# AkshayJha22/Cross-Sectional-Momentum-Strategy-Replication-Backtesting-Framework

Hardware: AMD Instinct MI355X
Metric: asset-periods backtested/sec (1/2/4/8 GPU) + % HBM peak BW; decile match % (higher is better)
Workload: dtype f64

## Files before the change

cross-sectional-momentum-strategy-replication-backtesting-framework_amd/csrc/scan.h:

```cpp
#pragma once
#include "csm_common.h"

struct ScanLane {
  double pff;
  double psff;
  int head;
  int prev;
};

__device__ __forceinline__ void scan_init(ScanLane& s, double* ring, int RS, int W,
                                          const double* __restrict__ carry, int64_t N,
                                          int64_t a, bool live) {
  if (live && carry) {
    for (int k = 0; k < W; ++k) ring[k * RS] = carry[(int64_t)k * N + a];
    s.pff = carry[(int64_t)W * N + a];
    s.psff = carry[(int64_t)(W + 1) * N + a];
  } else {
    for (int k = 0; k < W; ++k) ring[k * RS] = qnan();
    s.pff = qnan();
    s.psff = qnan();
  }
  s.head = 0;
  s.prev = -1;
}

__device__ __forceinline__ double ffill(double x, double last) { return isnan_d(x) ? last : x; }

__device__ __forceinline__ double price_step(double x, double& pff) {
  const double nx = ffill(x, pff);
  const double ret = nx / pff - 1.0;
  pff = nx;
  return ret;
}

__device__ __forceinline__ void lds_push(double* ring, int RS, int W, int& head, double fct) {
  ring[head * RS] = fct;
  head = (head + 1 == W) ? 0 : head + 1;
}

template <int JC = 0>
__device__ __forceinline__ double lds_prod(const double* ring, int RS, int W, int J, int idx) {
  double acc = ring[idx * RS];
  if constexpr (JC > 0) {
    double f[JC];
#pragma unroll
    for (int k = 1; k < JC; ++k) {
      idx = (idx + 1 == W) ? 0 : idx + 1;
      f[k] = ring[idx * RS];
    }
#pragma unroll
    for (int k = 1; k < JC; ++k) acc = acc * f[k];
  } else {
    for (int k = 1; k < J; ++k) {
      idx = (idx + 1 == W) ? 0 : idx + 1;
      acc = acc * ring[idx * RS];
    }
  }
  return acc;
}

template <int RW>
__device__ __forceinline__ void reg_push(double (&f)[RW], double fct, bool on = true) {
#pragma unroll
  for (int k = 0; k + 1 < RW; ++k) f[k] = on ? f[k + 1] : f[k];
  f[RW - 1] = on ? fct : f[RW - 1];
}

template <int RW>
__device__ __forceinline__ double reg_prod(const double (&f)[RW], int J) {
  double acc = f[0];
#pragma unroll
  for (int k = 1; k < RW; ++k)
    if (k < J) acc = acc * f[k];
  return acc;
}

template <int RW, bool FIX>
__device__ __forceinline__ double mj_window(const double (&f)[RW], int q, int lo, int hi) {
  if constexpr (FIX) {
    constexpr int Jq[4] = {3, 6, 9, 12};
    double acc = 0.0;
#pragma unroll
    for (int qq = 0; qq < 4; ++qq) {
      if (qq != q) continue;
      const int l = RW - Jq[qq] - 1;
      double a = f[l];
#pragma unroll
      for (int k = l + 1; k < RW - 1; ++k) a = a * f[k];
      acc = a;
    }
    return acc;
  }
  double acc = 1.0;
#pragma unroll
  for (int k = 0; k < RW; ++k) acc = (k >= lo && k < hi) ? acc * f[k] : acc;
  return acc;
}

__device__ __forceinline__ double subset_ret(double ps_new, double psff) {
  return ps_new / psff - 1.0;
}

template <class Settle>
__device__ __forceinline__ bool rank_step(double x, double mom, int m, double& psff, int& prev,
                                          Settle settle) {
  const bool ranked = !isnan_d(mom);
  const double ps_new = ffill(x, psff);
  if (prev >= 0) settle(prev, subset_ret(ps_new, psff));
  if (ranked) {
    psff = ps_new;
    prev = m;
    return false;
  }
  prev = -1;
  return true;
}

__device__ __forceinline__ double pending_finish(double x, double psff) {
  return is_absent(x) ? qnan() : subset_ret(ffill(x, psff), psff);
}

__device__ __forceinline__ void scan_finish(ScanLane& s, double* ring, int RS, int W, int64_t N,
                                            int64_t a, double* __restrict__ NR,
                                            const double* __restrict__ next_pm,
                                            double* __restrict__ carry_out) {
  if (s.prev >= 0)
    NR[(int64_t)s.prev * N + a] = next_pm ? pending_finish(next_pm[a], s.psff) : qnan();
  if (carry_out) {
    int idx = s.head;
    for (int k = 0; k < W; ++k) {
      carry_out[(int64_t)k * N + a] = ring[idx * RS];
      idx = (idx + 1 == W) ? 0 : idx + 1;
    }
    carry_out[(int64_t)W * N + a] = s.pff;
    carry_out[(int64_t)(W + 1) * N + a] = s.psff;
  }
}

template <int JC = 0>
__device__ __forceinline__ double lds_push_mom(ScanLane& s, double* ring, int RS, int W, int J,
                                               double fct) {
  lds_push(ring, RS, W, s.head, fct);
  return lds_prod<JC>(ring, RS, W, J, s.head) - 1.0;
}

template <class Ring>
__device__ __forceinline__ double scan_step_on(ScanLane& s, double x, int m, int64_t N, int64_t a,
                                               double* __restrict__ R, double* __restrict__ M,
                                               double* __restrict__ NR, Ring push_prod) {
  const double NaN = qnan();
  const int64_t o = (int64_t)m * N + a;
  if (is_absent(x)) {
    if (R) R[o] = NaN;
    M[o] = NaN;
    NR[o] = NaN;
    return NaN;
  }
  const double ret = price_step(x, s.pff);
  const double mom = push_prod(1.0 + ret);
  if (rank_step(x, mom, m, s.psff, s.prev,
                [&](int row, double nr) { NR[(int64_t)row * N + a] = nr; }))
    NR[o] = NaN;
  if (R) R[o] = ret;
  M[o] = mom;
  return mom;
}

__device__ __forceinline__ void store_pair(double* p, double v0, double v1) {
  *reinterpret_cast<double2*>(p) = make_double2(v0, v1);
}

__device__ __forceinline__ void store_next_ret_pair(double* __restrict__ NR, int64_t N,
                                                    int64_t a0, int64_t o, const int (&wp)[2],
                                                    const double (&vp)[2], const bool (&wc)[2]) {
  const double NaN = qnan();
  if (wp[0] >= 0 && wp[0] == wp[1]) {
    store_pair(NR + (int64_t)wp[0] * N + a0, vp[0], vp[1]);
  } else {
    if (wp[0] >= 0) NR[(int64_t)wp[0] * N + a0] = vp[0];
    if (wp[1] >= 0) NR[(int64_t)wp[1] * N + a0 + 1] = vp[1];
  }
  if (wc[0] && wc[1]) {
    store_pair(NR + o, NaN, NaN);
  } else {
    if (wc[0]) NR[o] = NaN;
    if (wc[1]) NR[o + 1] = NaN;
  }
}

__device__ __forceinline__ void chunk_range(int T_m, int G, int g, int& m0, int& m1) {
  const int base = T_m / G, rem = T_m % G;
  m0 = g * base + (g < rem ? g : rem);
  m1 = m0 + base + (g < rem ? 1 : 0);
}

template <int JC = 0>
__device__ __forceinline__ double scan_step(ScanLane& s, double x, int m, double* ring, int RS,
                                            int W, int J, int64_t N, int64_t a,
                                            double* __restrict__ R, double* __restrict__ M,
                                            double* __restrict__ NR) {
  return scan_step_on(s, x, m, N, a, R, M, NR,
                      [&](double fct) { return lds_push_mom<JC>(s, ring, RS, W, J, fct); });
}

template <int JC = 0>
__device__ __forceinline__ void scan_step_pair(ScanLane (&s)[2], const double (&x)[2], int m,
                                               double* ring0, int RS, int W, int J, int64_t N,
                                               int64_t a0, double* __restrict__ R,
                                               double* __restrict__ M, double* __restrict__ NR,
                                               double (&mom)[2]) {
  const double NaN = qnan();
  double ret[2];
  int wp[2];
  double vp[2];
  bool wc[2];
#pragma unroll
  for (int c = 0; c < 2; ++c) {
    wp[c] = -1;
    vp[c] = NaN;
    if (is_absent(x[c])) {
      ret[c] = NaN; mom[c] = NaN; wc[c] = true;
      continue;
    }
    ret[c] = price_step(x[c], s[c].pff);
    mom[c] = lds_push_mom<JC>(s[c], ring0 + c, RS, W, J, 1.0 + ret[c]);
    const bool ranked = !isnan_d(mom[c]);
    const double ps_new = ffill(x[c], s[c].psff);
    if (s[c].prev >= 0) { wp[c] = s[c].prev; vp[c] = subset_ret(ps_new, s[c].psff); }
    if (ranked) {
      s[c].psff = ps_new;
      s[c].prev = m;
      wc[c] = false;
    } else {
      s[c].prev = -1;
      wc[c] = true;
    }
  }
  const int64_t o = (int64_t)m * N + a0;
  if (R) store_pair(R + o, ret[0], ret[1]);
  store_pair(M + o, mom[0], mom[1]);
  store_next_ret_pair(NR, N, a0, o, wp, vp, wc);
}

__device__ __forceinline__ void scan_shadow(ScanLane& s, double x, int m, double* ring, int RS,
                                            int W, int J) {
  if (is_absent(x)) return;
  const double ret = price_step(x, s.pff);
  const double mom = lds_push_mom(s, ring, RS, W, J, 1.0 + ret);
  rank_step(x, mom, m, s.psff, s.prev, [](int, double) {});
}

template <int VEC> struct RowT;
template <> struct RowT<1> { typedef double T; };
template <> struct RowT<2> { typedef double2 T; };
__device__ __forceinline__ double comp(double v, int) { return v; }
__device__ __forceinline__ double comp(double2 v, int k) { return k == 0 ? v.x : v.y; }

template <int WR, int JC = 0>
__device__ __forceinline__ double scan_step_reg(ScanLane& s, double x, int m, double (&fr)[WR],
                                                int J, int64_t N, int64_t a,
                                                double* __restrict__ R, double* __restrict__ M,
                                                double* __restrict__ NR) {
  return scan_step_on(s, x, m, N, a, R, M, NR, [&](double fct) {
    reg_push(fr, fct);
    return reg_prod(fr, JC > 0 ? JC : J) - 1.0;
  });
}
```

cross-sectional-momentum-strategy-replication-backtesting-framework_amd/csrc/signal.hip:

```cpp
#include "csm_common.h"
#include "scan.h"
#include "shard.h"


#define PROBE_M 8
#define PROBE_DEN 8
__device__ __forceinline__ bool tail_probe(const double* __restrict__ P,
                                           const int64_t* __restrict__ month_start, int T_m,
                                           int64_t N, int64_t T_d) {
  static_assert(PROBE_M == 8, "the month spacing is a shift");
  const int lane = threadIdx.x & 63;
  const int64_t cs = N / 128;
  double x[PROBE_M][2];
  bool in[PROBE_M];
#pragma unroll
  for (int i = 0; i < PROBE_M; ++i) {
    const int m = (int)(((int64_t)(2 * i + 1) * T_m) >> 4);
    const int64_t d0 = month_start[m] < 0 ? 0 : month_start[m];
    const int64_t d1 = month_start[m + 1] < T_d ? month_start[m + 1] : T_d;
    in[i] = d1 > d0;
#pragma unroll
    for (int j = 0; j < 2; ++j)
      x[i][j] = in[i] ? P[(d1 - 1) * N + (2 * lane + j) * cs] : 0.0;
  }
  int gaps = 0, tot = 0;
#pragma unroll
  for (int i = 0; i < PROBE_M; ++i)
#pragma unroll
    for (int j = 0; j < 2; ++j) {
      gaps += __popcll(__ballot(in[i] && !(x[i][j] == x[i][j])));
      tot += in[i] ? 64 : 0;
    }
  return gaps * PROBE_DEN <= tot;
}

struct HaloArgs {
  int H, F, before, after;
  uint8_t* flags;
};
#define HALO_BATCH 8
template <int MAXD, int VEC, int NBUF, int BW, bool SH, bool BL, int JC = 0, bool HALO = false>
__global__ __launch_bounds__(64 * BW) void k_signal(
    const double* __restrict__ P, const int64_t* __restrict__ month_start, int T_m, int64_t N,
    int J, int skip, double* __restrict__ PMo, double* __restrict__ R, double* __restrict__ M,
    double* __restrict__ NR, const double* __restrict__ carry, const double* __restrict__ next_pm,
    double* __restrict__ carry_out, int64_t T_d, uint16_t* __restrict__ IDS, HaloArgs ha,
    int probe) {
  static_assert(!HALO || (SH && VEC == 2), "the halo prologue: shard passes, paired lanes");
  if (probe && tail_probe(P, month_start, T_m, N, T_d)) return;
  typedef typename RowT<VEC>::T VT;
  extern __shared__ __attribute__((aligned(16))) double ring_lds[];
  const int W = J + skip;
  const int tid = threadIdx.x;
  const int64_t a0 = ((int64_t)blockIdx.x * 64 * BW + tid) * VEC;
  const bool live = a0 < N;
  const int RS = 64 * VEC * BW;
  ScanLane sl[VEC];
  int* shc = reinterpret_cast<int*>(ring_lds + W * RS);
#pragma unroll
  for (int k = 0; k < VEC; ++k) {
    scan_init(sl[k], ring_lds + VEC * tid + k, RS, W, HALO ? nullptr : carry, N, a0 + k, live);
    if (SH) {
      shc[VEC * tid + k] = 0;
      shc[RS + VEC * tid + k] = -1;
      shc[2 * RS + VEC * tid + k] = -1;
    }
  }
  double npmh[VEC];
  if constexpr (HALO) {
    constexpr int HU = HALO_BATCH;
    const int64_t* ms = month_start;
    const int H = ha.H, F = ha.F, HF = H + F;
    const int64_t as = live ? a0 : 0;
    const int lane = tid & 63, wv = tid >> 6;
    const int64_t aw = a0 - 2 * lane;
    double* hpw = ring_lds + (size_t)W * RS + (size_t)(3 * RS) / 2;
    uint16_t* wl = reinterpret_cast<uint16_t*>(hpw + HU * RS) + wv * (HU * 128);
    int nh[VEC], fv[VEC], lv[VEC];
#pragma unroll
    for (int c = 0; c < VEC; ++c) { nh[c] = 0; fv[c] = -1; lv[c] = -1; npmh[c] = absent_val(); }
    for (int j0 = 0; j0 < HF; j0 += HU) {
      double2 xl[HU];
#pragma unroll
      for (int u = 0; u < HU; ++u) {
        const int j = j0 + u;
        const int m = j < H ? j : j + T_m;
        xl[u] = make_double2(absent_val(), absent_val());
        if (j < HF) {
          const int64_t d0 = ms[m], d1 = ms[m + 1];
          if (d1 > d0) xl[u] = *reinterpret_cast<const double2*>(P + (d1 - 1) * N + as);
        }
      }
      int nit = 0;
#pragma unroll
      for (int u = 0; u < HU; ++u) {
        *reinterpret_cast<double2*>(hpw + u * RS + 2 * tid) = xl[u];
#pragma unroll
        for (int c = 0; c < VEC; ++c) {
          const double x = comp(xl[u], c);
          const bool need = live && j0 + u < HF && !(x == x);
          const uint64_t mk = __ballot(need);
          if (need) wl[nit + lane_prefix(mk)] = (uint16_t)(u * 128 + 2 * lane + c);
          nit += __popcll(mk);
        }
      }
      __builtin_amdgcn_wave_barrier();
      for (int it0 = 0; it0 < nit; it0 += 128) {
        int item[2], u[2];
        int64_t d0[2], d1[2];
        double xs[2][HALO_WALK];
#pragma unroll
        for (int h = 0; h < 2; ++h) {
          const int it = it0 + 64 * h + lane;
          item[h] = it < nit ? (int)wl[it] : -1;
          u[h] = item[h] >> 7;
          const int j = j0 + (item[h] < 0 ? 0 : u[h]);
          const int m = j < H ? j : j + T_m;
          d0[h] = ms[m];
          d1[h] = ms[m + 1];
          const int64_t a = aw + (item[h] & 127);
#pragma unroll
          for (int k = 0; k < HALO_WALK; ++k) {
            const int64_t d = d1[h] - 2 - k;
            xs[h][k] = (item[h] >= 0 && d >= d0[h]) ? P[d * N + a] : absent_val();
          }
        }
#pragma unroll
        for (int h = 0; h < 2; ++h) {
          if (item[h] < 0) continue;
          const int64_t a = aw + (item[h] & 127);
          const double xlast = hpw[u[h] * RS + 128 * wv + (item[h] & 127)];
          bool p = !is_absent(xlast), got = false;
          double x = 0.0;
#pragma unroll
          for (int k = 0; k < HALO_WALK; ++k) {
            if (!got && xs[h][k] == xs[h][k]) { x = xs[h][k]; got = true; }
            p |= !is_absent(xs[h][k]);
          }
          if (!got && d1[h] - 1 - HALO_WALK > d0[h]) {
            const double y = halo_month_price(P, d0[h], d1[h] - 1 - HALO_WALK, N, a);
            if (y == y) { x = y; got = true; }
            p |= !is_absent(y);
          }
          hpw[u[h] * RS + 128 * wv + (item[h] & 127)] = got ? x : (p ? qnan() : absent_val());
        }
      }
      __syncthreads();
#pragma unroll
      for (int u = 0; u < HU; ++u) {
        const int j = j0 + u;
        if (j >= HF) break;
#pragma unroll
        for (int c = 0; c < VEC; ++c) {
          const double x = hpw[u * RS + 2 * tid + c];
          if (j < H) {
            if (live && !is_absent(x)) {
              if (!isnan_d(x)) { if (fv[c] < 0) fv[c] = nh[c]; lv[c] = nh[c]; }
              ++nh[c];
              scan_shadow(sl[c], x, j, ring_lds + VEC * tid + c, RS, W, J);
            }
          } else if (is_absent(npmh[c])) {
            npmh[c] = x;
          }
        }
      }
      __syncthreads();
    }
#pragma unroll
    for (int c = 0; c < VEC; ++c) {
      sl[c].prev = -1;
      uint8_t fl = 0;
      if (ha.before && !(fv[c] >= 0 && lv[c] - fv[c] >= W)) fl |= 1;
      if (ha.after && is_absent(npmh[c])) fl |= 2;
      if (live && ha.flags) ha.flags[a0 + c] = fl;
    }
    month_start += H;
  }
  const double* base = P + (live ? a0 : 0);
  const int64_t rstride = N;
  static_assert(!BL || VEC == 2, "buffer loads: paired lanes");
  const int voff = (int)((live ? a0 : 0) * 8);
  auto load_month = [&](VT (&buf)[MAXD], int mm) {
    mm = mm < T_m ? mm : T_m - 1;
    const int64_t f0 = month_start[mm], nn = month_start[mm + 1] - f0;
    if constexpr (BL) {
      typedef unsigned int u32x4 __attribute__((ext_vector_type(4)));
      const __amdgpu_buffer_rsrc_t rs = __builtin_amdgcn_make_buffer_rsrc(
          (void*)(P + f0 * N), (short)0, (int)(nn * N * 8), 0x00020000);
#pragma unroll
      for (int k = 0; k < MAXD; ++k) {
        const u32x4 w = __builtin_amdgcn_raw_buffer_load_b128(rs, voff + k * (int)(N * 8), 0, 0);
        buf[k] = *reinterpret_cast<const VT*>(&w);
      }
    } else {
      const int64_t pad = nn > 0 ? nn - 1 : (f0 > 0 ? -1 : 0);
#pragma unroll
      for (int k = 0; k < MAXD; ++k)
        buf[k] = *reinterpret_cast<const VT*>(base + (f0 + (k < nn ? k : pad)) * rstride);
    }
  };
  auto process = [&](const VT (&X)[MAXD], int m) {
    double pm[VEC];
    const int nnm = (int)(month_start[m + 1] - month_start[m]);
#pragma unroll
    for (int c = 0; c < VEC; ++c) {
      double last = 0.0;
      bool p = false, v = false;
#pragma unroll
      for (int k = 0; k < MAXD; ++k) {
        const double x = comp(X[k], c);
        const bool in = BL ? k < nnm : nnm > 0;
        const bool ok = in && x == x;
        p |= in && !is_absent(x);
        v |= ok;
        last = ok ? x : last;
      }
      pm[c] = p ? (v ? last : qnan()) : absent_val();
      if (SH && p) {
        int* q = shc + VEC * tid + c;
        q[0] += 1;
        if (q[RS] < 0) q[RS] = m;
        q[2 * RS] = m;
      }
    }
    if (live) {
      if (PMo && (!SH || shard_pm_kept(m, T_m, W))) {
        if (VEC == 2) *reinterpret_cast<double2*>(PMo + (int64_t)m * N + a0) = make_double2(pm[0], pm[VEC - 1]);
        else PMo[(int64_t)m * N + a0] = pm[0];
      }
      double mom[VEC];
      if constexpr (VEC == 2) {
        scan_step_pair<JC>(reinterpret_cast<ScanLane (&)[2]>(sl), reinterpret_cast<const double (&)[2]>(pm),
                       m, ring_lds + VEC * tid, RS, W, J, N, a0, R, M, NR,
                       reinterpret_cast<double (&)[2]>(mom));
      } else {
#pragma unroll
        for (int c = 0; c < VEC; ++c)
          mom[c] = scan_step(sl[c], pm[c], m, ring_lds + VEC * tid + c, RS, W, J, N, a0 + c, R, M, NR);
      }
      if (IDS) {
        if (VEC == 2)
          *reinterpret_cast<uint32_t*>(IDS + (int64_t)m * N + a0) =
              csm_fid(mom[0]) | (csm_fid(mom[VEC - 1]) << 16);
        else
          IDS[(int64_t)m * N + a0] = (uint16_t)csm_fid(mom[0]);
      }
    }
  };
  static_assert(NBUF == 2 || NBUF == 4, "two or four month buffers");
  VT A[MAXD], B[MAXD];
  if (NBUF == 2) {
    load_month(A, 0);
    for (int m = 0; m < T_m; m += 2) {
      load_month(B, m + 1);
      process(A, m);
      load_month(A, m + 2);
      if (m + 1 < T_m) process(B, m + 1);
    }
  } else {
    VT C[MAXD], D[MAXD];
    load_month(A, 0);
    load_month(B, 1);
    load_month(C, 2);
    for (int m = 0; m < T_m; m += 4) {
      load_month(D, m + 3);
      process(A, m);
      load_month(A, m + 4);
      if (m + 1 < T_m) process(B, m + 1);
      load_month(B, m + 5);
      if (m + 2 < T_m) process(C, m + 2);
      load_month(C, m + 6);
      if (m + 3 < T_m) process(D, m + 3);
    }
  }
  if (live) {
#pragma unroll
    for (int k = 0; k < VEC; ++k) {
      if constexpr (HALO) {
        if (sl[k].prev >= 0)
          NR[(int64_t)sl[k].prev * N + a0 + k] = pending_finish(npmh[k], sl[k].psff);
      } else {
        scan_finish(sl[k], ring_lds + VEC * tid + k, RS, W, N, a0 + k, NR, next_pm,
                    SH ? nullptr : carry_out);
      }
      if (SH) {
        const int* q = shc + VEC * tid + k;
        carry_out[a0 + k] = (double)q[0];
        carry_out[N + a0 + k] = (double)sl[k].prev;
        carry_out[2 * N + a0 + k] = sl[k].psff;
        carry_out[3 * N + a0 + k] = (double)q[RS];
        carry_out[4 * N + a0 + k] = (double)q[2 * RS];
      }
    }
  }
}

#define TAIL_U 8
#define TAIL_BACK 3

template <int MAXD, int BW, int JC>
__global__ __launch_bounds__(64 * BW) void k_signal_tail(
    const double* __restrict__ P, const int64_t* __restrict__ month_start, int T_m, int64_t N,
    int J, int skip, double* __restrict__ PMo, double* __restrict__ R, double* __restrict__ M,
    double* __restrict__ NR, const double* __restrict__ carry, const double* __restrict__ next_pm,
    double* __restrict__ carry_out, int64_t T_d, uint16_t* __restrict__ IDS,
    int probe) {
  if (probe && !tail_probe(P, month_start, T_m, N, T_d)) return;
  extern __shared__ __attribute__((aligned(16))) double ring_lds[];
  constexpr int U = TAIL_U, RS = 64 * BW, WA = 64;
  const int W = J + skip;
  const int tid = threadIdx.x, lane = tid & 63, wv = tid >> 6;
  const int64_t a0 = (int64_t)blockIdx.x * RS + tid;
  const bool live = a0 < N;
  const int64_t as = live ? a0 : 0;
  const int64_t aw = a0 - lane;
  const int64_t* ms = month_start;
  double* hp = ring_lds + (size_t)W * RS;
  double* hpw = hp + WA * wv;
  uint16_t* wl = reinterpret_cast<uint16_t*>(hp + U * RS) + wv * (2 * U * WA);
  uint16_t* wl2 = wl + U * WA;
  ScanLane sl;
  scan_init(sl, ring_lds + tid, RS, W, carry, N, a0, live);
  if (aw >= N) return;

  auto month_rows = [&](int m, int64_t& d0, int64_t& d1) {
    d0 = ms[m];
    d1 = ms[m + 1];
    d0 = d0 < 0 ? 0 : d0;
    d1 = d1 < T_d ? d1 : T_d;
  };
  auto load_last = [&](double (&xl)[U], int m0) {
#pragma unroll
    for (int u = 0; u < U; ++u) {
      xl[u] = absent_val();
      if (m0 + u < T_m) {
        int64_t d0, d1;
        month_rows(m0 + u, d0, d1);
        if (d1 > d0) xl[u] = P[(d1 - 1) * N + as];
      }
    }
  };
  auto fold = [&](double y, double& x, bool& got, bool& p) {
    if (!got && y == y) { x = y; got = true; }
    p |= !is_absent(y);
  };
  constexpr int K = MAXD - 1;
  struct Walk {
    int item, u, col;
    int64_t d0, d1;
    bool act;
  };
  auto issue = [&](auto& xs, Walk& w, const uint16_t* list, int it, int n, int m0) {
    constexpr int KK = sizeof(xs) / sizeof(double);
    w.act = it < n;
    w.item = w.act ? (int)list[it] : 0;
    w.u = w.item / WA;
    w.col = w.item % WA;
    month_rows(m0 + w.u, w.d0, w.d1);
    const int64_t a = aw + w.col;
#pragma unroll
    for (int k = 0; k < KK; ++k) {
      const int64_t d = w.d1 - 2 - k;
      xs[k] = (w.act && d >= w.d0) ? P[d * N + a] : absent_val();
    }
  };
  auto finish_back = [&](const double (&xs)[TAIL_BACK], const Walk& w, int& nb) {
    bool p = true, got = false;
    double x = 0.0;
#pragma unroll
    for (int k = 0; k < TAIL_BACK; ++k) fold(xs[k], x, got, p);
    const bool more = w.act && !got && w.d1 - 2 - TAIL_BACK >= w.d0;
    if (w.act && !more) hpw[w.u * RS + w.col] = got ? x : qnan();
    const uint64_t mk = __ballot(more);
    if (more) wl2[nb + lane_prefix(mk)] = (uint16_t)w.item;
    nb += __popcll(mk);
  };
  auto finish_month = [&](const double (&xs)[K], const Walk& w) {
    bool p = !is_absent(hpw[w.u * RS + w.col]), got = false;
    double x = 0.0;
#pragma unroll
    for (int k = 0; k < K; ++k) fold(xs[k], x, got, p);
    if (w.act) hpw[w.u * RS + w.col] = got ? x : (p ? qnan() : absent_val());
  };
  auto walk_months = [&](int i0, int n, int m0) {
    double XS[K], XT[K];
    Walk wb, wc;
    const bool two = i0 + 64 < n;
    issue(XS, wb, wl2, i0 + lane, n, m0);
    if (two) issue(XT, wc, wl2, i0 + 64 + lane, n, m0);
    finish_month(XS, wb);
    if (two) finish_month(XT, wc);
  };

  double xa[U], xb[U];
  load_last(xa, 0);
  for (int m0 = 0; m0 < T_m; m0 += U) {
    load_last(xb, m0 + U);
    int na = 0, nb = 0;
#pragma unroll
    for (int u = 0; u < U; ++u) {
      hp[u * RS + tid] = xa[u];
      bool in = false;
      if (m0 + u < T_m) {
        int64_t d0, d1;
        month_rows(m0 + u, d0, d1);
        in = d1 > d0;
      }
      const double x = xa[u];
      const bool need = live && in && !(x == x);
      const bool nb_ = need && is_absent(x), na_ = need && !nb_;
      const uint64_t mka = __ballot(na_), mkb = __ballot(nb_);
      const int item = u * WA + lane;
      if (na_) wl[na + lane_prefix(mka)] = (uint16_t)item;
      if (nb_) wl2[nb + lane_prefix(mkb)] = (uint16_t)item;
      na += __popcll(mka);
      nb += __popcll(mkb);
    }
    __builtin_amdgcn_wave_barrier();
    if (na + nb > 0) {
      double xs[TAIL_BACK];
      Walk wa;
      int db = nb < 128 ? nb : 128;
      issue(xs, wa, wl, lane, na, m0);
      walk_months(0, db, m0);
      finish_back(xs, wa, nb);
      for (int it0 = 64; it0 < na; it0 += 64) {
        issue(xs, wa, wl, it0 + lane, na, m0);
        finish_back(xs, wa, nb);
      }
      __builtin_amdgcn_wave_barrier();
      for (; db < nb; db += 128) walk_months(db, nb, m0);
    }
    __builtin_amdgcn_wave_barrier();
#pragma unroll 1
    for (int u = 0; u < U; ++u) {
      const int m = m0 + u;
      if (m >= T_m) break;
      if (!live) continue;
      const double pm = hp[u * RS + tid];
      if (PMo) PMo[(int64_t)m * N + a0] = pm;
      const double mom = scan_step<JC>(sl, pm, m, ring_lds + tid, RS, W, J, N, a0, R, M, NR);
      if (IDS) IDS[(int64_t)m * N + a0] = (uint16_t)csm_fid(mom);
    }
    __builtin_amdgcn_wave_barrier();
#pragma unroll
    for (int u = 0; u < U; ++u) xa[u] = xb[u];
  }
  if (live) scan_finish(sl, ring_lds + tid, RS, W, N, a0, NR, next_pm, carry_out);
}

static int g_tune_signal_vec = 2;
static int g_tune_signal_bwf = 0;
static int g_tune_signal_tail = 2;
static int g_tune_signal_j12 = 1;
#define SIGNAL_BWF_MIN_N (180 * 512)
static const TuneKnob g_knobs[] = {
    {"signal_vec", &g_tune_signal_vec, [](int v) { return v == 1 || v == 2; }},
    {"signal_bwf", &g_tune_signal_bwf, [](int v) { return v == 0 || v == 1 || v == 4; }},
    {"signal_j12", &g_tune_signal_j12, [](int v) { return v == 0 || v == 1; }},
    {"signal_tail", &g_tune_signal_tail, [](int v) { return v >= 0 && v <= 2; }},
};
int csm_tune_signal(const char* key, int value) { return tune_set(g_knobs, key, value); }

int signal_launch(csm_ctx* ctx, const char* who, const double* P, int64_t T_d, int64_t N,
                  const int64_t* month_start, int32_t T_m, int32_t max_month_days, int32_t J,
                  int32_t skip, double* PM, double* R, double* M, double* NR, const double* carry,
                  const double* next_pm, double* carry_out, bool sh, uint16_t* ids,
                  const HaloArgs* halo) {
  int r = prep(ctx);
  if (r) return r;
  if (sh && (!PM || !carry_out || T_m < 1))
    return set_err(ctx, CSM_E_INVAL, "%s: a shard pass needs PM and state, and at least one month",
                   who);
  if (!P || !month_start || !M || !NR || N <= 0 || T_d < 0 || T_m < 0 || J < 1 || skip < 0 ||
      J + skip > 256 || max_month_days < 1)
    return set_err(ctx, CSM_E_INVAL, "%s: bad arguments (N=%lld T_m=%d J=%d skip=%d)", who,
                   (long long)N, T_m, J, skip);
  if (max_month_days > 32)
    return set_err(ctx, CSM_E_INVAL, "%s: months longer than 32 days are not supported "
                   "(use csm_month_end + csm_momentum)", who);
  if (T_m == 0) return CSM_OK;
  if (T_d == 0)
    return set_err(ctx, CSM_E_INVAL, "%s: %d months and no day row", who, T_m);
  const int W = J + skip;
  const bool can2 = (N % 2 == 0) && aligned16(P) && (!PM || aligned16(PM)) && aligned16(M) &&
                    aligned16(NR) && (!R || aligned16(R));
  const int vec = (g_tune_signal_vec == 1 || !can2) ? 1 : 2;
  const size_t tlds = (size_t)(W + TAIL_U) * 128 * sizeof(double) + (size_t)2 * TAIL_U * 128 * sizeof(uint16_t);
  int tail = (!sh && !halo && can2 && tlds <= 160 * 1024) ? g_tune_signal_tail : 0;
  if (tail == 2 && N < (int64_t)SIGNAL_BWF_MIN_N) tail = 1;
  int probe_ = tail == 2;
  if (tail != 0) {
    const bool d23 = max_month_days <= 23, j12 = J == 12;
    const void* fn =
        d23 ? (j12 ? (const void*)k_signal_tail<23, 2, 12> : (const void*)k_signal_tail<23, 2, 0>)
            : (j12 ? (const void*)k_signal_tail<32, 2, 12> : (const void*)k_signal_tail<32, 2, 0>);
    if (tlds > 65536)
      HIP_CHECK(ctx, hipFuncSetAttribute(fn, hipFuncAttributeMaxDynamicSharedMemorySize, (int)tlds));
    const unsigned blocks = (unsigned)((N + 127) / 128);
    int T_m_ = T_m, J_ = J, skip_ = skip;
    int64_t N_ = N, T_d_ = T_d;
    void* args[] = {(void*)&P, (void*)&month_start, &T_m_, &N_, &J_, &skip_, (void*)&PM, (void*)&R,
                    (void*)&M, (void*)&NR, (void*)&carry, (void*)&next_pm, (void*)&carry_out, &T_d_,
                    (void*)&ids, &probe_};
    HIP_CHECK(ctx, hipLaunchKernel(fn, dim3(blocks), dim3(128), args, tlds, ctx->stream));
    LAUNCH_CHECK(ctx, who);
    if (tail == 1) return CSM_OK;
  }
  const bool fits4 = vec == 2 && max_month_days <= 23 && N * 8 * 32 < ((int64_t)1 << 31);
  const bool wide4 = fits4 && (g_tune_signal_bwf == 4 ||
                               (g_tune_signal_bwf == 0 && N >= (int64_t)SIGNAL_BWF_MIN_N));
  const int bw = wide4 ? 4 : 1;
  const size_t lds = (size_t)W * 64 * vec * bw * sizeof(double) +
                     (sh ? (size_t)3 * 64 * vec * bw * sizeof(int) : 0) +
                     (halo ? (size_t)HALO_BATCH * 64 * vec * bw * sizeof(double) +
                             (size_t)bw * HALO_BATCH * 128 * sizeof(uint16_t) : 0);
  const unsigned blocks = (unsigned)((N / vec + 64 * bw - 1) / (64 * bw));
  const void* fn = nullptr;
#define SIG1(V, SH_)                                                                            \
  (max_month_days <= 23 && V == 2 ? (const void*)k_signal<23, V, 4, 1, SH_, false>              \
   : max_month_days <= 24         ? (const void*)k_signal<24, V, 4, 1, SH_, false>              \
                                  : (const void*)k_signal<32, V, 4, 1, SH_, false>)
  const bool j12 = sh && J == 12 && g_tune_signal_j12;
  if (halo && !(sh && wide4))
    return set_err(ctx, CSM_E_INVAL, "%s: the fused halo prologue runs in the wide shard kernel "
                   "(even N >= %d, months of <= 23 days); use csm_shard_halo + "
                   "csm_signal_shard_halo", who, SIGNAL_BWF_MIN_N);
  if (halo)
    fn = j12 ? (const void*)k_signal<23, 2, 2, 4, true, true, 12, true>
             : (const void*)k_signal<23, 2, 2, 4, true, true, 0, true>;
  else if (wide4 && j12)
    fn = (const void*)k_signal<23, 2, 2, 4, true, true, 12>;
  else if (wide4)
    fn = sh ? (const void*)k_signal<23, 2, 2, 4, true, true> : (const void*)k_signal<23, 2, 2, 4, false, true>;
  else if (vec == 2)
    fn = sh ? SIG1(2, true) : SIG1(2, false);
  else
    fn = sh ? SIG1(1, true) : SIG1(1, false);
#undef SIG1
  if (lds > 65536)
    HIP_CHECK(ctx, hipFuncSetAttribute(fn, hipFuncAttributeMaxDynamicSharedMemorySize, (int)lds));
  {
    int T_m_ = T_m, J_ = J, skip_ = skip;
    int64_t N_ = N, T_d_ = T_d;
    HaloArgs ha = halo ? *halo : HaloArgs{0, 0, 0, 0, nullptr};
    void* args[] = {(void*)&P, (void*)&month_start, &T_m_, &N_, &J_, &skip_, (void*)&PM, (void*)&R,
                    (void*)&M, (void*)&NR, (void*)&carry, (void*)&next_pm, (void*)&carry_out, &T_d_,
                    (void*)&ids, (void*)&ha, &probe_};
    HIP_CHECK(ctx, hipLaunchKernel(fn, dim3(blocks), dim3(64 * bw), args, lds, ctx->stream));
  }
  LAUNCH_CHECK(ctx, who);
  return CSM_OK;
}

extern "C" {

int csm_signal(csm_ctx* ctx, const double* P, int64_t T_d, int64_t N, const int64_t* month_start,
               int32_t T_m, int32_t max_month_days, int32_t J, int32_t skip, double* PM, double* R,
               double* M, double* NR, const double* carry, const double* next_pm,
               double* carry_out) {
  return signal_launch(ctx, "csm_signal", P, T_d, N, month_start, T_m, max_month_days, J,
                       skip, PM, R, M, NR, carry, next_pm, carry_out);
}

int csm_signal_ids(csm_ctx* ctx, const double* P, int64_t T_d, int64_t N,
                   const int64_t* month_start, int32_t T_m, int32_t max_month_days,
                   int32_t min_month_days, int32_t J, int32_t skip, double* PM, double* R,
                   double* M, double* NR, uint16_t* ids) {
  if (!ids || (N % 4) != 0 || ((uintptr_t)ids & 7u) != 0)
    return set_err(ctx, CSM_E_INVAL, "csm_signal_ids: ids must be non-NULL and 8-B aligned, N %% 4 == 0 "
                   "(N=%lld)", (long long)N);
  (void)min_month_days;
  return signal_launch(ctx, "csm_signal_ids", P, T_d, N, month_start, T_m, max_month_days, J,
                       skip, PM, R, M, NR, nullptr, nullptr, nullptr, false, ids);
}

int csm_signal_shard(csm_ctx* ctx, const double* P, int64_t T_d, int64_t N,
                     const int64_t* month_start, int32_t T_m, int32_t max_month_days, int32_t J,
                     int32_t skip, double* PM, double* R, double* M, double* NR, double* state) {
  return signal_launch(ctx, "csm_signal_shard", P, T_d, N, month_start, T_m,
                       max_month_days, J, skip, PM, R, M, NR, nullptr, nullptr, state, true);
}

int csm_signal_shard_ids(csm_ctx* ctx, const double* P, int64_t T_d, int64_t N,
                         const int64_t* month_start, int32_t T_m, int32_t max_month_days,
                         int32_t J, int32_t skip, double* PM, double* R, double* M, double* NR,
                         double* state, uint16_t* ids) {
  if (!ids || (N % 4) != 0 || ((uintptr_t)ids & 7u) != 0)
    return set_err(ctx, CSM_E_INVAL, "csm_signal_shard_ids: needs ids, N %% 4 == 0, 8-B aligned ids");
  return signal_launch(ctx, "csm_signal_shard_ids", P, T_d, N, month_start, T_m,
                       max_month_days, J, skip, PM, R, M, NR, nullptr, nullptr, state, true, ids);
}

int csm_signal_halo(csm_ctx* ctx, const double* P, int64_t T_d, int64_t N,
                    const int64_t* month_start, int32_t H, int32_t T_m, int32_t F, int32_t before,
                    int32_t after, int32_t max_month_days, int32_t J, int32_t skip, double* PM,
                    double* R, double* M, double* NR, double* state, uint16_t* ids,
                    uint8_t* flags) {
  if (!flags || H < 0 || F < 0 || F > 8 || J + skip > 64)
    return set_err(ctx, CSM_E_INVAL, "csm_signal_halo: bad arguments (flags [N], H >= 0, "
                   "0 <= F <= 8, J + skip <= 64)");
  if (ids && ((N % 4) != 0 || ((uintptr_t)ids & 7u) != 0))
    return set_err(ctx, CSM_E_INVAL, "csm_signal_halo: ids need N %% 4 == 0, 8-B alignment");
  const HaloArgs ha{H, F, before ? 1 : 0, after ? 1 : 0, flags};
  return signal_launch(ctx, "csm_signal_halo", P, T_d, N, month_start, T_m, max_month_days, J,
                       skip, PM, R, M, NR, nullptr, nullptr, state, true, ids, &ha);
}

int csm_signal_shard_halo(csm_ctx* ctx, const double* P, int64_t T_d, int64_t N,
                          const int64_t* month_start, int32_t T_m, int32_t max_month_days,
                          int32_t J, int32_t skip, const double* carry, const double* next_pm,
                          double* PM, double* R, double* M, double* NR, double* state,
                          uint16_t* ids) {
  if (!carry || !next_pm)
    return set_err(ctx, CSM_E_INVAL, "csm_signal_shard_halo: needs the halo's carry and next_pm");
  if (ids && ((N % 4) != 0 || ((uintptr_t)ids & 7u) != 0))
    return set_err(ctx, CSM_E_INVAL, "csm_signal_shard_halo: ids need N %% 4 == 0, 8-B alignment");
  return signal_launch(ctx, "csm_signal_shard_halo", P, T_d, N, month_start, T_m, max_month_days,
                       J, skip, PM, R, M, NR, carry, next_pm, state, true, ids);
}

}
```

Measured before the change: 829.8 billion.

## Mirror LDS momentum ring and reuse price return for subset settlement

Doubles the LDS ring so each push writes the factor twice, letting the trailing J-product read contiguous slots without modular index wrapping. The settle step reuses the already-computed price return when the forward-filled and subset prices are bitwise equal, and does the division only under a wave ballot when some lane diverges. An OUT template flag drops the PM/R output paths when those outputs are null. The cost is a doubled ring footprint in LDS, which may lower occupancy or push large windows past the LDS limit, plus an extra LDS store per push.

```diff
diff --git a/cross-sectional-momentum-strategy-replication-backtesting-framework_amd/csrc/scan.h b/cross-sectional-momentum-strategy-replication-backtesting-framework_amd/csrc/scan.h
--- a/cross-sectional-momentum-strategy-replication-backtesting-framework_amd/csrc/scan.h
+++ b/cross-sectional-momentum-strategy-replication-backtesting-framework_amd/csrc/scan.h
@@ -59,6 +59,42 @@
   return acc;
 }
 
+template <int RS>
+__device__ __forceinline__ void lds2_fill(double* ring, int W) {
+  for (int k = 0; k < W; ++k) ring[(k + W) * RS] = ring[k * RS];
+}
+
+template <int RS>
+__device__ __forceinline__ void lds2_push(double* ring, int W, int& head, double fct) {
+  double* p = ring + head * RS;
+  p[0] = fct;
+  p[W * RS] = fct;
+  head = (head + 1 == W) ? 0 : head + 1;
+}
+
+template <int JC, int RS>
+__device__ __forceinline__ double lds2_prod(const double* ring, int J, int head) {
+  const double* p = ring + head * RS;
+  double acc = p[0];
+  if constexpr (JC > 0) {
+    double f[JC];
+#pragma unroll
+    for (int k = 1; k < JC; ++k) f[k] = p[k * RS];
+#pragma unroll
+    for (int k = 1; k < JC; ++k) acc = acc * f[k];
+  } else {
+    for (int k = 1; k < J; ++k) acc = acc * p[k * RS];
+  }
+  return acc;
+}
+
+template <int JC, int RS>
+__device__ __forceinline__ double lds2_push_mom(ScanLane& s, double* ring, int W, int J,
+                                                double fct) {
+  lds2_push<RS>(ring, W, s.head, fct);
+  return lds2_prod<JC, RS>(ring, J, s.head) - 1.0;
+}
+
 template <int RW>
 __device__ __forceinline__ void reg_push(double (&f)[RW], double fct, bool on = true) {
 #pragma unroll
@@ -107,6 +143,26 @@
   const bool ranked = !isnan_d(mom);
   const double ps_new = ffill(x, psff);
   if (prev >= 0) settle(prev, subset_ret(ps_new, psff));
+  if (ranked) {
+    psff = ps_new;
+    prev = m;
+    return false;
+  }
+  prev = -1;
+  return true;
+}
+
+template <class Settle>
+__device__ __forceinline__ bool rank_step_same(double x, double mom, int m, double ret, bool same,
+                                               double& psff, int& prev, Settle settle) {
+  const bool ranked = !isnan_d(mom);
+  const double ps_new = ffill(x, psff);
+  const bool div = prev >= 0 && !same;
+  double nr = ret;
+  if (__ballot(div)) {
+    if (div) nr = subset_ret(ps_new, psff);
+  }
+  if (prev >= 0) settle(prev, nr);
   if (ranked) {
     psff = ps_new;
     prev = m;
@@ -201,6 +257,30 @@
                                             double* __restrict__ NR) {
   return scan_step_on(s, x, m, N, a, R, M, NR,
                       [&](double fct) { return lds_push_mom<JC>(s, ring, RS, W, J, fct); });
+}
+
+template <int JC, int RS, bool WR>
+__device__ __forceinline__ double scan_step_mirror(ScanLane& s, double x, int m, double* ring,
+                                                   int W, int J, int64_t N, int64_t a,
+                                                   double* __restrict__ R, double* __restrict__ M,
+                                                   double* __restrict__ NR) {
+  const double NaN = qnan();
+  const int64_t o = (int64_t)m * N + a;
+  if (is_absent(x)) {
+    if (WR && R) R[o] = NaN;
+    M[o] = NaN;
+    NR[o] = NaN;
+    return NaN;
+  }
+  const bool same = __double_as_longlong(s.pff) == __double_as_longlong(s.psff);
+  const double ret = price_step(x, s.pff);
+  const double mom = lds2_push_mom<JC, RS>(s, ring, W, J, 1.0 + ret);
+  if (rank_step_same(x, mom, m, ret, same, s.psff, s.prev,
+                     [&](int row, double nr) { NR[(int64_t)row * N + a] = nr; }))
+    NR[o] = NaN;
+  if (WR && R) R[o] = ret;
+  M[o] = mom;
+  return mom;
 }
 
 template <int JC = 0>
diff --git a/cross-sectional-momentum-strategy-replication-backtesting-framework_amd/csrc/signal.hip b/cross-sectional-momentum-strategy-replication-backtesting-framework_amd/csrc/signal.hip
--- a/cross-sectional-momentum-strategy-replication-backtesting-framework_amd/csrc/signal.hip
+++ b/cross-sectional-momentum-strategy-replication-backtesting-framework_amd/csrc/signal.hip
@@ -298,7 +298,7 @@
 #define TAIL_U 8
 #define TAIL_BACK 3
 
-template <int MAXD, int BW, int JC>
+template <int MAXD, int BW, int JC, bool OUT>
 __global__ __launch_bounds__(64 * BW) void k_signal_tail(
     const double* __restrict__ P, const int64_t* __restrict__ month_start, int T_m, int64_t N,
     int J, int skip, double* __restrict__ PMo, double* __restrict__ R, double* __restrict__ M,
@@ -315,12 +315,13 @@
   const int64_t as = live ? a0 : 0;
   const int64_t aw = a0 - lane;
   const int64_t* ms = month_start;
-  double* hp = ring_lds + (size_t)W * RS;
+  double* hp = ring_lds + (size_t)2 * W * RS;
   double* hpw = hp + WA * wv;
   uint16_t* wl = reinterpret_cast<uint16_t*>(hp + U * RS) + wv * (2 * U * WA);
   uint16_t* wl2 = wl + U * WA;
   ScanLane sl;
   scan_init(sl, ring_lds + tid, RS, W, carry, N, a0, live);
+  lds2_fill<RS>(ring_lds + tid, W);
   if (aw >= N) return;
 
   auto month_rows = [&](int m, int64_t& d0, int64_t& d1) {
@@ -438,8 +439,8 @@
       if (m >= T_m) break;
       if (!live) continue;
       const double pm = hp[u * RS + tid];
-      if (PMo) PMo[(int64_t)m * N + a0] = pm;
-      const double mom = scan_step<JC>(sl, pm, m, ring_lds + tid, RS, W, J, N, a0, R, M, NR);
+      if (OUT && PMo) PMo[(int64_t)m * N + a0] = pm;
+      const double mom = scan_step_mirror<JC, RS, OUT>(sl, pm, m, ring_lds + tid, W, J, N, a0, R, M, NR);
       if (IDS) IDS[(int64_t)m * N + a0] = (uint16_t)csm_fid(mom);
     }
     __builtin_amdgcn_wave_barrier();
@@ -486,15 +487,17 @@
   const bool can2 = (N % 2 == 0) && aligned16(P) && (!PM || aligned16(PM)) && aligned16(M) &&
                     aligned16(NR) && (!R || aligned16(R));
   const int vec = (g_tune_signal_vec == 1 || !can2) ? 1 : 2;
-  const size_t tlds = (size_t)(W + TAIL_U) * 128 * sizeof(double) + (size_t)2 * TAIL_U * 128 * sizeof(uint16_t);
+  const size_t tlds = (size_t)(2 * W + TAIL_U) * 128 * sizeof(double) + (size_t)2 * TAIL_U * 128 * sizeof(uint16_t);
   int tail = (!sh && !halo && can2 && tlds <= 160 * 1024) ? g_tune_signal_tail : 0;
   if (tail == 2 && N < (int64_t)SIGNAL_BWF_MIN_N) tail = 1;
   int probe_ = tail == 2;
   if (tail != 0) {
     const bool d23 = max_month_days <= 23, j12 = J == 12;
-    const void* fn =
-        d23 ? (j12 ? (const void*)k_signal_tail<23, 2, 12> : (const void*)k_signal_tail<23, 2, 0>)
-            : (j12 ? (const void*)k_signal_tail<32, 2, 12> : (const void*)k_signal_tail<32, 2, 0>);
+#define TAIL(OUT_)                                                                              \
+  (d23 ? (j12 ? (const void*)k_signal_tail<23, 2, 12, OUT_> : (const void*)k_signal_tail<23, 2, 0, OUT_>) \
+       : (j12 ? (const void*)k_signal_tail<32, 2, 12, OUT_> : (const void*)k_signal_tail<32, 2, 0, OUT_>))
+    const void* fn = (PM || R) ? TAIL(true) : TAIL(false);
+#undef TAIL
     if (tlds > 65536)
       HIP_CHECK(ctx, hipFuncSetAttribute(fn, hipFuncAttributeMaxDynamicSharedMemorySize, (int)tlds));
     const unsigned blocks = (unsigned)((N + 127) / 128);
```

New measurement: 864.0 billion, median of 6. +4.1%, better.
